# xuhao1/TaichiSLAM

Hardware: AMD Instinct MI355X
Metric: depth-frames/s integrated (640x480->512^3 TSDF) (higher is better)
Workload: dtype f16 storage / f32 + int64 fixed-point arithmetic; 1 GPU; BASELINE configs[1]: single 640x480 u16 depth stream (sphere room r=3 m, 1 deg/frame) -> DenseTSDF 512^3 / 2 cm, recast_step 2, max_ray 5 m; one stream+submap per GPU

## Files before the change

### taichislam_amd/csrc/tsl_integrate.hip

```cpp
#include "tsl_tsdf.hpp"
#include <hip/hip_ext.h>

namespace tsl {

#ifdef TSL_TIMING
#define TSL_T0() const int _wv = (blockIdx.x * (int)blockDim.x + (int)threadIdx.x) >> 6
#define TSL_TICK(F, k) do { long long _n = wall_clock64(); if (lane_id() == 0 && _wv < 16384) (F).dbg[_wv * 16 + (k)] = _n; } while (0)
#else
#define TSL_T0() do {} while (0)
#define TSL_TICK(F, k) do {} while (0)
#endif

#define SCATTER_TILE 4096

struct RayRegs { float pf0, pf1, pf2, d0, d1, d2, P0, P1, P2, w; long long qden; int n; };

__device__ __forceinline__ uint32_t wave_min_u32(uint32_t v)
{
    for (int d = 32; d > 0; d >>= 1) { const uint32_t o = (uint32_t)__shfl_xor((int)v, d); v = o < v ? o : v; }
    return v;
}
__device__ __forceinline__ RayRegs make_ray(const uint4 rec, int n, const FrameParams& P)
{
    RayRegs R;
    R.n = n;
    R.pf0 = h2f((h16)(rec.x & 0xffffu)); R.pf1 = h2f((h16)(rec.x >> 16)); R.pf2 = h2f((h16)(rec.y & 0xffffu));
    R.d0 = h2f((h16)(rec.y >> 16)); R.d1 = h2f((h16)(rec.z & 0xffffu)); R.d2 = h2f((h16)(rec.z >> 16));
    R.w = __uint_as_float(rec.w);
    R.qden = to_fix(R.w);
    R.P0 = R.pf0 + P.T[0]; R.P1 = R.pf1 + P.T[1]; R.P2 = R.pf2 + P.T[2];
    return R;
}
template <bool WITH_N = true>
__device__ __forceinline__ RayRegs load_ray(const FrameDev& F, const FrameParams& P, int r) { return make_ray(F.rayA[r], WITH_N ? F.rayN[r] : 0, P); }
__device__ __forceinline__ void step_voxel(const RayRegs& R, const FrameParams& P, int j, float* x, int* xi)
{
    const float jf = (float)j;
    x[0] = (R.d0 * jf) * P.vs + P.T[0]; x[1] = (R.d1 * jf) * P.vs + P.T[1]; x[2] = (R.d2 * jf) * P.vs + P.T[2];
    xi[0] = rnd_i(div_vs(x[0], P.vs, P.rvs, P.fastdiv)); xi[1] = rnd_i(div_vs(x[1], P.vs, P.rvs, P.fastdiv)); xi[2] = rnd_i(div_vs(x[2], P.vs, P.rvs, P.fastdiv));
}
__device__ __forceinline__ long long step_term(const RayRegs& R, const float* x)
{
    const float v0 = R.P0 - x[0], v1 = R.P1 - x[1], v2 = R.P2 - x[2];
    const float s2 = (v0 * v0 + v1 * v1) + v2 * v2;
    const float dist = s2 >= 1.2621774483536189e-29f ? sqrt_rn_norm(s2) : sqrt_rn(s2);
    const float dot = (v0 * R.pf0 + v1 * R.pf1) + v2 * R.pf2;
    const float sd = dist * (float)sgn_f(dot);
    return to_fix_wave(R.w * sd);
}
template <bool COOP = true>
__device__ __forceinline__ void mark_occupied(const MapDev& M, const FrameParams& P, const RayRegs& R)
{
    const int oi = rnd_i(div_vs(R.P0, P.vs, P.rvs, P.fastdiv)), oj = rnd_i(div_vs(R.P1, P.vs, P.rvs, P.fastdiv)), ok = rnd_i(div_vs(R.P2, P.vs, P.rvs, P.fastdiv));
    if (in_volume(M, oi, oj, ok)) {
        int l; const int b = brick_of(M, oi, oj, ok, &l);
        const int p = pool_claim<COOP>(M, P.slot, b);
        if (p >= 0) M.occ[(size_t)p * TSL_BRK3 + l] = 1;
    }
}
template <bool COOP = true>
__device__ __forceinline__ int frame_slot_slow(const MapDev& M, const FrameDev& F, int s, int b)
{
    const int sl = COOP ? claim_index(F.slot_tab + b, &F.counters[1], F.max_frame_bricks) : claim_index_1(F.slot_tab + b, &F.counters[1], F.max_frame_bricks);
    if (sl >= 0) {
        const int p = pool_claim<COOP>(M, s, b);
        if (p >= 0) { F.touched[sl] = p; F.touched_b[sl] = b; }
        else return -1;
    } else frame_fail(M, F, 2);
// ... 12 lines not shown
    const h16 Tn = f2h((h2f(hmul(T0, W0)) + num) / (h2f(W0) + den));
    float wn = h2f(W0) + den; if (TSL_WMAX < wn) wn = TSL_WMAX;
    return (uint32_t)Tn | ((uint32_t)f2h(wn) << 16);
}
__device__ __forceinline__ uint32_t apply_update_f(uint32_t old, float num, float den)
{
    const h16 T0 = (h16)(old & 0xffffu), W0 = (h16)(old >> 16);
    const h16 Tn = f2h((h2f(hmul(T0, W0)) + num) / (h2f(W0) + den));
    float wn = h2f(W0) + den; if (TSL_WMAX < wn) wn = TSL_WMAX;
    return (uint32_t)Tn | ((uint32_t)f2h(wn) << 16);
}

template <int VARIANT>
__global__ void __launch_bounds__(256) k_integrate(MapDev M, FrameDev F, const FrameParams* __restrict__ Pp)
{
    const FrameParams& P = *Pp;
    const int split = P.split;
    const int gid = blockIdx.x * 256 + threadIdx.x;
    const int r = gid / split, sub = gid - r * split;
    const int nrays = *F.nrays;
    const bool live = r < nrays;
    long long n_ok = 0, n_oob = 0;
    RayRegs R; R.n = 0; R.qden = 0;
    if (live) { R = load_ray(F, P, r); if (sub == 0) mark_occupied(M, P, R); }
    int cur_b = -1; unsigned long long* cur_acc = nullptr;
    int nmax = R.n;
    if (VARIANT == 1) { for (int d = 32; d > 0; d >>= 1) { int o = __shfl_xor(nmax, d); nmax = o > nmax ? o : nmax; } }
    const int iters = (nmax + split - 1) / split;
    for (int it = 0; it < iters; ++it) {
        const int j = 1 + sub + it * split;
        const bool act = live && j <= R.n;
        unsigned long long* dst = nullptr;
        long long qn = 0;
        if (act) {
            float x[3]; int xi[3];
            step_voxel(R, P, j, x, xi);
            if (in_volume(M, xi[0], xi[1], xi[2])) {
                qn = step_term(R, x);
                int l; const int b = brick_of(M, xi[0], xi[1], xi[2], &l);
                if (b != cur_b) { cur_b = b; const int sl = frame_slot(M, F, P.slot, b); cur_acc = sl >= 0 ? F.acc + (size_t)sl * (TSL_BRK3 * 2) : nullptr; }
                if (cur_acc) { dst = cur_acc + (size_t)l * 2; ++n_ok; }
            } else ++n_oob;
        }
        if (VARIANT == 1) {
            const unsigned long long m = __ballot(dst != nullptr);
            if (m) {
                const int leader = (int)__builtin_ctzll(m);
                const unsigned long long lead = __shfl((unsigned long long)dst, leader);
                const bool same = (dst == nullptr) || ((unsigned long long)dst == lead);
                if (__all(same)) {
                    const long long sn = wave_sum_ll(dst ? qn : 0), sdn = wave_sum_ll(dst ? R.qden : 0);
// ... 37 lines not shown
            const int l = q * 256 + threadIdx.x;
            if (a[q].y != 0ull) {
                tw[l] = apply_update(old[q], (long long)a[q].x, (long long)a[q].y);
                obs[l] = 1;
                acc[l] = make_ulonglong2(0ull, 0ull);
                ++uniq;
            }
        }
    }
    for (int sl = blockIdx.x * 256 + threadIdx.x; sl < ntouched; sl += gridDim.x * 256) F.slot_tab[F.touched_b[sl]] = TSL_EMPTY;
    uniq = wave_sum_ll(uniq);
    if (lane_id() == 0 && uniq) atomic_add_i64(&F.stats->unique, uniq);
    if (!list && blockIdx.x == 0 && threadIdx.x == 0) F.stats->bricks = ntouched;
}

__device__ __forceinline__ int axis_coord(float d, float T, const FrameParams& P, int j) { return rnd_i(div_vs((d * (float)j) * P.vs + T, P.vs, P.rvs, P.fastdiv)); }
__device__ __forceinline__ int axis_cell(int c, int h, int N, int nb) { const int u = c + h; return u < 0 ? -1 : (u >= N ? nb : (u >> 4)); }

__device__ __forceinline__ int next_axis_event(float d, float inv_d, float T, const FrameParams& P, float t_over_vs, int j, int jb, int cell, int h, int N, int nb)
{
    if (j >= jb) return jb + 1;
    int bound;
    bool up;
    if (d > 0.0f) { if (cell >= nb) return jb + 1; up = true; bound = (cell < 0 ? 0 : min((cell + 1) * 16, N)) - h; }
    else if (d < 0.0f) { if (cell < 0) return jb + 1; up = false; bound = (cell >= nb ? N - 1 : cell * 16 - 1) - h; }
    else return jb + 1;
    const float est = ((float)bound + (up ? -0.5f : 0.5f) - t_over_vs) * inv_d;
    int e = (int)fminf(fmaxf(ceilf(est), (float)(j + 1)), (float)jb);
    #define TSL_PRED(q) (up ? (axis_coord(d, T, P, (q)) >= bound) : (axis_coord(d, T, P, (q)) <= bound))
    if (TSL_PRED(e)) { while (e - 1 > j && TSL_PRED(e - 1)) --e; }
    else { ++e; while (e <= jb && !TSL_PRED(e)) ++e; }
    #undef TSL_PRED
    return e;
}

#define LH_SIZE 1024
#define LH_EMPTY (-1)
template <int LOG2 = 10>
__device__ __forceinline__ int lh_slot(int* keys, int b)
{
    unsigned h = ((unsigned)b * 2654435761u) >> (32 - LOG2);
    for (int probe = 0; probe < (1 << LOG2); ++probe) {
        const int k = keys[h];
        if (k == b) return (int)h;
        if (k == LH_EMPTY) { const int old = atomicCAS(&keys[h], LH_EMPTY, b); if (old == LH_EMPTY || old == b) return (int)h; }
        h = (h + 1) & ((1u << LOG2) - 1u);
    }
    return -1;
}

#define SEG_RAY_SLOTS 16
#define SEG_LH_LOG2 9
#define SEG_LH (1 << SEG_LH_LOG2)
template <bool FUSED>
__global__ void __launch_bounds__(256) k_segments(MapDev M, BatchDev B)
{
    if ((int)blockIdx.y >= B.n) return;
    const FrameDev& F = B.f[blockIdx.y];
    const FrameParams& P = *B.p[blockIdx.y];
    __shared__ int s_key[SEG_LH];
    __shared__ int s_cnt[SEG_LH];
    TSL_T0();
    TSL_TICK(F, 8);
    for (int i = threadIdx.x; i < SEG_LH; i += 256) { s_key[i] = LH_EMPTY; s_cnt[i] = 0; }
    __syncthreads();
    TSL_TICK(F, 0);

    const int split = P.split;
    const int gid = blockIdx.x * 256 + threadIdx.x;
    const int r = gid / split, sub = gid - r * split;
    const int nrays = FUSED ? F.counters[6] : *F.nrays;
    long long n_ok = 0, n_oob = 0;
    const bool working = __any(r < nrays);
    const int spl = SEG_RAY_SLOTS / split;
    unsigned long long* myseg = F.seg + (size_t)gid * spl;
    int nslot = 0;
    bool ok = r < nrays;
    uint4 rec = make_uint4(0, 0, 0, 0);
    int nsteps = 0;
    if (FUSED) {
        const int lane = threadIdx.x & 63;
        bool big = false;
        int gn = 0, sl = 0;
// ... 11 lines not shown
                uint32_t id[H_INL] = { w0.w, w1.x, w1.y, w1.z, w1.w, w2.x, w2.y, w2.z, w2.w, w3.x, w3.y, w3.z, w3.w };
                uint2 pl[H_INL];
#pragma unroll
                for (int q = 0; q < H_INL; ++q) {
                    if (q >= gn) id[q] = 0xffffffffu;
                    pl[q] = q < gn ? F.pix[id[q]] : make_uint2(0u, 0u);
                }
                PixAcc A = {};
                for (int k = 0; k < gn; ++k) {
                    uint32_t best = 0xffffffffu; uint2 bp = make_uint2(0u, 0u);
#pragma unroll
                    for (int q = 0; q < H_INL; ++q) { const bool t = id[q] < best; best = t ? id[q] : best; bp.x = t ? pl[q].x : bp.x; bp.y = t ? pl[q].y : bp.y; }
#pragma unroll
                    for (int q = 0; q < H_INL; ++q) id[q] = id[q] == best ? 0xffffffffu : id[q];
                    if (k == 0) first = best;
                    if (P.tex) acc_colour(P, F, best, A);
                    acc_payload(bp, A);
                }
                ok = finish_ray(P, F, A, first, &rec, &nsteps);
            }
        }
        for (unsigned long long bm = __ballot(big); bm; bm &= bm - 1ull) {
            const int src = (int)__builtin_ctzll(bm);
            const int n = __shfl(gn, src), sl0 = __shfl(sl, src);
            const unsigned long long vk = ((unsigned long long)(uint32_t)__shfl((int)(vkey >> 32), src) << 32) | (unsigned long long)(uint32_t)__shfl((int)(uint32_t)vkey, src);
            const int nblk = (n + H_INL - 1) / H_INL;
            const uint32_t hmask = (1u << P.hlog2) - 1u;
            auto find_block = [&](int bq) -> int {
                if (bq == 0) return sl0;
                const unsigned long long k2 = h_key(vk, bq);
                uint32_t h = h_hash64(k2, P.hlog2);
                for (uint32_t probe = 0; probe <= hmask; ++probe) {
                    const unsigned long long cur = F.htab[h].key;
                    if (cur == k2) return (int)h;
// ... 11 lines not shown
                uint32_t best = 0xffffffffu;
                for (int bq = lane; bq < nblk; bq += 64) {
                    const int hs = bq == lane ? mine : find_block(bq);
                    if (hs < 0) continue;
                    const int cb = min(H_INL, n - bq * H_INL);
                    const uint32_t* ids = F.htab[hs].pix;
                    for (int q = 0; q < cb; ++q) { const uint32_t v = ids[q]; if ((long long)v > last && v < best) best = v; }
                }
                best = wave_min_u32(best);
                if (best == 0xffffffffu) break;
                if (k == 0) f0 = best;
                acc_pixel(P, F, best, A);
                last = (long long)best;
            }
            uint4 rc; int ns = 0;
            const bool k2 = A.cnt == n && finish_ray(P, F, A, f0, &rc, &ns, lane == src);
            if (lane == src) { rec = rc; nsteps = ns; ok = k2; first = f0; }
        }
        if (r < nrays && sub == 0) {
            F.rayA[r] = rec; F.rayFirst[r] = first;
            if (P.seq) {
                uint32_t u[3];
#pragma unroll
                for (int a = 0; a < 3; ++a) {
                    unsigned long long x = (vkey >> (2 - a)) & 0x1249249249249249ull;
                    x = (x | (x >> 2)) & 0x10c30c30c30c30c3ull; x = (x | (x >> 4)) & 0x100f00f00f00f00full; x = (x | (x >> 8)) & 0x1f0000ff0000ffull;
                    x = (x | (x >> 16)) & 0x1f00000000ffffull; x = (x | (x >> 32)) & 0x1fffffull;
                    u[a] = (uint32_t)x;
                }
                const unsigned long long nblk = (unsigned long long)(P.pcl_ext / P.pcl_blk), blk = (unsigned long long)P.pcl_blk;
                const unsigned long long kb = ((u[0] / P.pcl_blk) * nblk + (u[1] / P.pcl_blk)) * nblk + (u[2] / P.pcl_blk);
                const unsigned long long kl = ((u[0] % P.pcl_blk) * blk + (u[1] % P.pcl_blk)) * blk + (u[2] % P.pcl_blk);
                reinterpret_cast<unsigned long long*>(F.keys)[r] = kb * blk * blk * blk + kl;
                F.rayN[r] = ok ? nsteps : 0;
            }
        }
        block_count_add(&F.stats->v_pcl, r < nrays && sub == 0);
        block_count_add(&F.stats->v_skipped, r < nrays && sub == 0 && !ok);
        if (gid == 0) *F.nrays = nrays;
        const int src = lane - sub;
        rec.x = (uint32_t)__shfl((int)rec.x, src); rec.y = (uint32_t)__shfl((int)rec.y, src); rec.z = (uint32_t)__shfl((int)rec.z, src); rec.w = (uint32_t)__shfl((int)rec.w, src);
        nsteps = __shfl(nsteps, src);
        ok = __shfl((int)ok, src) != 0;
    }
    if (ok) {
        const RayRegs R = FUSED ? make_ray(rec, nsteps, P) : load_ray(F, P, r);
        if (sub == 0) mark_occupied(M, P, R);
        TSL_TICK(F, 1);
        const int len = (R.n + split - 1) / split;
        const int ja = 1 + sub * len, jb = min(R.n, ja + len - 1);
        const float d[3] = { R.d0, R.d1, R.d2 };
        const float id[3] = { __builtin_amdgcn_rcpf(R.d0), __builtin_amdgcn_rcpf(R.d1), __builtin_amdgcn_rcpf(R.d2) };
        const float tv[3] = { P.T[0] / P.vs, P.T[1] / P.vs, P.T[2] / P.vs };
        const int hh[3] = { M.hN, M.hN, M.hNz }, NN[3] = { M.N, M.N, M.Nz }, nb[3] = { M.nbx, M.nbx, M.nbz };
        if (ja <= jb) {
            int cell[3], ev[3];
#pragma unroll
            for (int a = 0; a < 3; ++a) {
                cell[a] = axis_cell(axis_coord(d[a], P.T[a], P, ja), hh[a], NN[a], nb[a]);
                ev[a] = next_axis_event(d[a], id[a], P.T[a], P, tv[a], ja, jb, cell[a], hh[a], NN[a], nb[a]);
            }
            int j = ja;
            while (j <= jb) {
                const int e = min(min(ev[0], ev[1]), ev[2]);
                const bool inside = cell[0] >= 0 && cell[0] < nb[0] && cell[1] >= 0 && cell[1] < nb[1] && cell[2] >= 0 && cell[2] < nb[2];
                if (inside) {
                    const int b = (cell[0] * M.nbx + cell[1]) * M.nbz + cell[2];
                    n_ok += e - j;
                    for (int j0 = j; j0 < e; j0 += SEG_MAX_CNT) {
                        const int cnt = min(e - j0, SEG_MAX_CNT);
                        const unsigned long long en = ((unsigned long long)b << STG_B_SHIFT) | ((unsigned long long)r << (SEG_CNT_BITS + SEG_J_BITS)) |
                                                      ((unsigned long long)j0 << SEG_CNT_BITS) | (unsigned long long)cnt;
                        bool stored = true;
                        if (nslot < spl) myseg[nslot++] = en;
                        else {
// ... 3 lines not shown
                        if (stored) {
                            const int hs = lh_slot<SEG_LH_LOG2>(s_key, b);
                            if (hs >= 0) atomicAdd(&s_cnt[hs], 1);
                            else if (__hip_atomic_fetch_add(&F.bhist[b], 1, __ATOMIC_RELAXED, __HIP_MEMORY_SCOPE_AGENT) == 0) {
                                const int q = __hip_atomic_fetch_add(&F.counters[1], 1, __ATOMIC_RELAXED, __HIP_MEMORY_SCOPE_AGENT);
                                if (q < F.max_frame_bricks) F.act_b[q] = b; else frame_fail(M, F, 2);
                            }
                        }
                    }
                } else n_oob += e - j;
                j = e;
                if (j > jb) break;
#pragma unroll
                for (int a = 0; a < 3; ++a) if (ev[a] == j) {
                    cell[a] += d[a] > 0.0f ? 1 : -1;
                    ev[a] = next_axis_event(d[a], id[a], P.T[a], P, tv[a], j, jb, cell[a], hh[a], NN[a], nb[a]);
                }
            }
        }
    }
    if (r < nrays) for (int q = nslot; q < spl; ++q) myseg[q] = ~0ull;
    TSL_TICK(F, 2);
    __syncthreads();
    TSL_TICK(F, 3);
    TSL_TICK(F, 5);
    for (int i = threadIdx.x; i < SEG_LH; i += 256) {
        const int c = s_cnt[i];
        const int b = c ? s_key[i] : 0;
        const bool first = c && __hip_atomic_fetch_add(&F.bhist[b], c, __ATOMIC_RELAXED, __HIP_MEMORY_SCOPE_AGENT) == 0;
        const int q = wave_reserve(&F.counters[1], first);
        if (first) { if (q < F.max_frame_bricks) F.act_b[q] = b; else frame_fail(M, F, 2); }
// ... 14 lines not shown
        }
        __syncthreads();
        if (threadIdx.x == 0) {
            if (s_steps[0]) atomic_add_i64(&F.stats->steps, s_steps[0]);
            if (s_steps[1]) atomic_add_i64(&F.stats->steps_oob, s_steps[1]);
        }
    }
}

__device__ __forceinline__ int plan_class(int w) { return w >= 2560 ? 0 : (w >= 1280 ? 1 : (w >= 512 ? 2 : 3)); }
__global__ void __launch_bounds__(256) k_plan(MapDev M, BatchDev B, int psegs, int unit_max, int unit_half)
{
    if ((int)blockIdx.y >= B.n) return;
    const int y = blockIdx.y;
    const FrameDev& F = B.f[y];
    const int listed = F.counters[1];
    const int nact = min(listed, F.max_frame_bricks);
    if ((int)blockIdx.x * 256 >= nact && blockIdx.x) return;
    const int i = blockIdx.x * 256 + threadIdx.x;
    int v = 0, b = 0, np = 0, pcls = -1, ucls = -1, tm = 0, wb = 0, tmu = 0, tmp = 0, wu = 0;
    if (i < nact) {
        b = F.act_b[i];
        v = F.bhist[b];
        int vq[TSL_NB];
#pragma unroll
        for (int q = 0; q < TSL_NB; ++q) { vq[q] = q < B.n ? B.f[q].bhist[b] : 0; if (vq[q] > 0) tm |= 1 << q; wb += vq[q]; }
        if (wb > unit_max) { tmp = tm; }
        else if (wb > unit_half) {
            int acc = 0;
#pragma unroll
            for (int q = 0; q < TSL_NB; ++q) if ((tm >> q) & 1) { if (2 * acc < wb) { tmu |= 1 << q; wu += vq[q]; } else tmp |= 1 << q; acc += vq[q]; }
        } else { tmu = tm; wu = wb; }
        if (tmu && (tmu & -tmu) == (1 << y)) ucls = plan_class(wu);
        if (((tmp >> y) & 1) && v > 0) { np = (v + psegs - 1) / psegs; pcls = plan_class((v + np - 1) / np); }
    }
    const int off = block_reserve_n(&F.counters[3], v);
    const int s0 = block_reserve_n(&B.f[0].counters[HDR_SLAB], np);
    int p0 = 0, u0 = 0;
    for (int c = 0; c < PLAN_NCLS; ++c) {
        const int q = block_reserve_n(&F.counters[HDR_PARTS + c], pcls == c ? np : 0); if (pcls == c) p0 = q;
        const int u = block_reserve_n(&B.f[0].counters[HDR_UNITS + c], ucls == c ? 1 : 0); if (ucls == c) u0 = u;
    }
    if (i < nact) {
        F.boffset[b] = off;
        F.bnseg[b] = v;
        const int pool = (np || ucls >= 0) ? pool_claim<false>(M, B.p[y]->slot, b) : -1;
        if (ucls >= 0) {
            if (u0 < B.f[0].unit_cap) B.f[0].unit_tab[(size_t)ucls * B.f[0].unit_cap + u0] = make_int4(b, wu, pool, tmu);
            else for (int q = 0; q < B.n; ++q) if ((tm >> q) & 1) frame_fail(M, B.f[q], 2);
        }
        if (np && pool >= 0) {
            if ((tmp & -tmp) == (1 << y)) {
                const int hi = __hip_atomic_fetch_add(&B.f[0].counters[HDR_HEAVY], 1, __ATOMIC_RELAXED, __HIP_MEMORY_SCOPE_AGENT);
                if (hi < B.f[0].max_frame_bricks) B.f[0].heavy_tab[hi] = make_int4(b, pool, tmp, 0);
                else for (int q = 0; q < B.n; ++q) if ((tm >> q) & 1) frame_fail(M, B.f[q], 2);
            }
            if (s0 + np > F.max_frame_bricks || np >= (1 << PART_NP_BITS) || p0 + np > F.part_cap) frame_fail(M, F, 2);
            else {
                F.bslab[b] = s0 | (np << SLAB_SLOT_BITS);
                const int per = (v + np - 1) / np;
                int4* tab = F.part_tab + (size_t)pcls * F.part_cap;
                for (int k = 0; k < np; ++k) {
                    const int pos = k * per, n = min(v, pos + per) - pos;
                    tab[p0 + k] = make_int4(off + pos, (int)((uint32_t)n | ((uint32_t)np << 16)), pool, s0 + k);
                }
            }
        }
    }
    if (i == 0) { F.stats->bricks = listed; if (listed > F.max_frame_bricks) frame_fail(M, F, 2); }
}

__global__ void __launch_bounds__(256) k_scatter(BatchDev B)
{
    if ((int)blockIdx.y >= B.n) return;
    const FrameDev& F = B.f[blockIdx.y];
    __shared__ int s_key[LH_SIZE];
    __shared__ int s_cnt[LH_SIZE];
    __shared__ int s_base[LH_SIZE];
    if (B.p[blockIdx.y]->group) {
        const int na = F.counters[6], nx = F.counters[7];
        for (int i = blockIdx.x * 256 + threadIdx.x; i < na + nx; i += gridDim.x * 256) {
            HSlot* const hs = F.htab + (i < na ? F.act[i] : F.actx[i - na]);
            hs->key = H_EMPTY; hs->cnt = 0;
        }
    }
    const int total = (int)min((long long)*F.nrays * SEG_RAY_SLOTS + F.counters[2], (long long)F.seg_cap);
    const int ntiles = (total + SCATTER_TILE - 1) / SCATTER_TILE;
    for (int tile = blockIdx.x; tile < ntiles; tile += gridDim.x) {
        for (int i = threadIdx.x; i < LH_SIZE; i += 256) { s_key[i] = LH_EMPTY; s_cnt[i] = 0; }
        __syncthreads();
        const int t0 = tile * SCATTER_TILE;
        unsigned long long key[SCATTER_TILE / 256]; int rank[SCATTER_TILE / 256]; int hs[SCATTER_TILE / 256];
#pragma unroll
        for (int q = 0; q < SCATTER_TILE / 256; ++q) {
            const int i = t0 + q * 256 + threadIdx.x;
            rank[q] = -1; hs[q] = -1;
            if (i < total) {
                key[q] = F.seg[i];
                if (key[q] != ~0ull) {
                    const int b = (int)(key[q] >> STG_B_SHIFT);
                    hs[q] = lh_slot<10>(s_key, b);
                    if (hs[q] >= 0) rank[q] = atomicAdd(&s_cnt[hs[q]], 1);
                    else rank[q] = F.boffset[b] + __hip_atomic_fetch_add(&F.bcursor[b], 1, __ATOMIC_RELAXED, __HIP_MEMORY_SCOPE_AGENT);
                }
            }
        }
        __syncthreads();
        for (int i = threadIdx.x; i < LH_SIZE; i += 256) {
            const int c = s_cnt[i];
            if (c) { const int b = s_key[i]; s_base[i] = F.boffset[b] + __hip_atomic_fetch_add(&F.bcursor[b], c, __ATOMIC_RELAXED, __HIP_MEMORY_SCOPE_AGENT); }
        }
        __syncthreads();
#pragma unroll
        for (int q = 0; q < SCATTER_TILE / 256; ++q)
            if (rank[q] >= 0) F.seg_sorted[(hs[q] >= 0 ? s_base[hs[q]] : 0) + rank[q]] = key[q];
        __syncthreads();
    }
}

#ifdef TSL_NOSWZ
__device__ __forceinline__ int acc_swz5(int l) { return l; }
#else
__device__ __forceinline__ int acc_swz5(int l) { return l ^ (((l >> 8) ^ (l >> 5)) & 31); }
#endif
struct StepK { float vs, rvs, T0, T1, T2; int hN, hNz; };
// ... 188 lines not shown
        if (threadIdx.x < 64) s_bin[threadIdx.x] = 0;
        __syncthreads();
        TSL_PRIME(0, f)
    }
    uint32_t old[VPT];
    uint32_t vmask = 0u;
    bool have_old = false;
    for (;;) {
        const int* const it = s_it[slot];
        const int slot1 = slot == 2 ? 0 : slot + 1, slot2 = slot == 0 ? 2 : slot - 1;
        const bool unit = uni(it[IT_UNIT]) != 0;
        const int p = uni(it[IT_POOL]), rk = uni(it[IT_SLAB]);
        const uint32_t fmask = (uint32_t)uni(it[IT_FMASK]);
        const int n_f = uni(it[IT_N + f]);
        const FrameDev& F = B.f[f];
        const FrameParams& P = *B.p[f];
        const StepK K = { P.vs, P.rvs, P.T[0], P.T[1], P.T[2], M.hN, M.hNz };
        const uint32_t later = fmask >> (f + 1);
        const bool first_frame = (fmask & ((1u << f) - 1u)) == 0u, last_frame = later == 0u;
        const bool first_step = first_frame && c == 0;
        const int nseg = min(CSEGS, n_f - c * CSEGS);
        const bool last_chunk = (c + 1) * CSEGS >= n_f;
        const bool last_step = last_chunk && last_frame;
        int known = max(1, (n_f + CSEGS - 1) / CSEGS) - 1 - c + steps_of(slot, later << (f + 1));
        if (n_known >= 1) known += steps_of(slot1, (uint32_t)uni(s_it[slot1][IT_FMASK]));
        const bool do_claim = !exhausted && n_known < 2 && known <= 1;
        if (do_claim && threadIdx.x == 0) s_claim[0] = __hip_atomic_fetch_add(claim, 1, __ATOMIC_RELAXED, __HIP_MEMORY_SCOPE_AGENT);
#ifdef TSL_TIMING
        long long* const _rec = F.dbg + 131072 + (size_t)blockIdx.x * 128 + (size_t)(t < 16 ? t : 15) * 8;
        if (threadIdx.x == 0 && first_step) { _rec[0] = wall_clock64(); _rec[1] = (unit ? 1 : 0) | (uni(it[IT_NP]) << 8) | ((long long)fmask << 32); _rec[2] = 0; _rec[5] = 0; }
        if (threadIdx.x == 0 && c == 0) _rec[2] += n_f;
// ... 15 lines not shown
#pragma unroll
        for (int q = 0; q < SPT; ++q) { const int i = q * NT + threadIdx.x; kn[q] = i < nsegn ? Fx.seg_sorted[offx + i] : 0ull; }
        const uint32_t* const twr = M.tw + (size_t)(p >= 0 ? p : 0) * TSL_BRK3;
        if (first_step) { have_old = false; vmask = 0u; }
        if (!TEX && unit && p >= 0 && first_step) {
#pragma unroll
            for (int q = 0; q < VPT; ++q) old[q] = twr[q * NT + threadIdx.x];
            have_old = true;
        }
#pragma unroll
        for (int q = 0; q < SPT; ++q) {
            const int i = q * NT + ((q & 1) ? NT - 1 - (int)threadIdx.x : (int)threadIdx.x);
            if (i >= nseg) continue;
            const unsigned long long key = kk[q];
            const int cnt = (int)(key & ((1u << SEG_CNT_BITS) - 1)), j0 = (int)((key >> SEG_CNT_BITS) & ((1u << SEG_J_BITS) - 1));
            const RayRegs R = make_ray(recs[q], 0, P);
            const uint32_t wid = wids[q];
#ifndef TSL_EXP_STAGGER
#define TSL_EXP_STAGGER 27
#endif
            int off = ((int)((threadIdx.x * (unsigned)TSL_EXP_STAGGER) & 63u) * cnt) >> 6;
            for (int s = 0; s < cnt; s += 2) {
                const int ja = j0 + off; off = (off + 1 == cnt) ? 0 : off + 1;
                const int jb = j0 + off; off = (off + 1 == cnt) ? 0 : off + 1;
                int la, lb; float qa, qb;
                step_eval<FASTDIV>(R, K, ja, &la, &qa);
                step_eval<FASTDIV>(R, K, jb, &lb, &qb);
                long long na = (long long)(int)qa, nb = (long long)(int)qb;
                if (__builtin_expect(__any(!(fabsf(qa) < 2147483648.0f) || !(fabsf(qb) < 2147483648.0f)), 0)) { na = __float2ll_rn(qa); nb = __float2ll_rn(qb); }
                atomicAdd(&S_NUM(la), (unsigned long long)na);
                atomicAdd(&S_DEN(la), (unsigned long long)R.qden);
// ... 218 lines not shown
}

int check_variant2(tsl_tsdf* m)
{
    TSL_REQUIRE(m->F.max_frame_bricks <= 4096 && m->P.max_steps_f < (float)(1 << SEG_J_BITS) && m->F.max_points < (1 << STG_RAY_BITS) && m->nb3 < (1 << 24) && 3 * m->pcl_bits <= H_BLOCK_SHIFT,
                "variant 2: ray too long / too many points / too many bricks for the segment key (use variant 1)");
    return TSL_OK;
}

int launch_segments(tsl_tsdf* m, const BatchDev& B, const FrameParams* hp, int total, hipStream_t st)
{
    const FrameParams& P = hp[0];
    if (P.variant != 2) return TSL_OK;
    const int iblocks = (int)(((int64_t)total * P.split + 255) / 256);
    prof_begin(m, TSL_K_SEGMENTS, st);
    if (P.group) hipLaunchKernelGGL(k_segments<true>, dim3(iblocks, B.n), dim3(256), 0, st, m->M, B);
    else hipLaunchKernelGGL(k_segments<false>, dim3(iblocks, B.n), dim3(256), 0, st, m->M, B);
    prof_end(m, st);
    int unit_max = m->unit_max <= m->unit_floor ? m->unit_max : std::max(m->unit_floor, (int)((long long)m->unit_max * B.n / TSL_NB));
    int unit_half = std::min(unit_max, m->unit_half <= 2048 ? m->unit_half : std::max(2048, (int)((long long)m->unit_half * B.n / TSL_NB)));
    if (P.seq && m->seq_impl) unit_max = unit_half = 1 << 30;
    prof_begin(m, TSL_K_BIN, st);
    hipLaunchKernelGGL(k_plan, dim3((B.f[0].max_frame_bricks + 255) / 256, B.n), dim3(256), 0, st, m->M, B, m->chunks * m->wg * m->spt, unit_max, unit_half);
    hipLaunchKernelGGL(k_scatter, dim3(256, B.n), dim3(256), 0, st, B);
    prof_end(m, st);
    return TSL_OK;
}

int launch_brick(tsl_tsdf* m, const BatchDev& B, const FrameParams& P, int kind, hipStream_t st, hipEvent_t start, hipEvent_t stop)
{
    const int bg = kind == 2 ? m->pgrid : (B.n <= 2 ? (m->bgrid + 1) / 2 : (kind == 1 ? m->ugrid : m->bgrid));
#define TSL_LAUNCH_IB(TEXV, FD) do { \
        if (m->wg == 512 && m->spt == 2 && !TEXV) hipExtLaunchKernelGGL((k_integrate_batch<false, FD, 512, 2, 4>), dim3((2 * m->ncu * bg + 99) / 100), dim3(512), 0, st, start, stop, 0, m->M, B, kind); \
        else if (m->wg == 512) hipExtLaunchKernelGGL((k_integrate_batch<TEXV, FD, 512, 4, 2>), dim3((m->ncu * bg + 99) / 100), dim3(512), 0, st, start, stop, 0, m->M, B, kind); \
        else hipExtLaunchKernelGGL((k_integrate_batch<TEXV, FD, 256, 4, (TEXV ? 1 : 2)>), dim3(((TEXV ? 1 : 2) * m->ncu * bg + 99) / 100), dim3(256), 0, st, start, stop, 0, m->M, B, kind); } while (0)
    if (P.tex) { if (P.fastdiv) TSL_LAUNCH_IB(true, true); else TSL_LAUNCH_IB(true, false); }
    else { if (P.fastdiv) TSL_LAUNCH_IB(false, true); else TSL_LAUNCH_IB(false, false); }
#undef TSL_LAUNCH_IB
    TSL_HIP(hipGetLastError());
// ... 35 lines not shown
```

### taichislam_amd/csrc/tsl_tsdf.hip

```cpp
#include "tsl_tsdf.hpp"
#include <rocprim/rocprim.hpp>
#include <algorithm>
#include <cmath>
#include <cstdio>
#include <cstdlib>
#include <cstring>
#include <mutex>

namespace tsl {

static thread_local std::string g_err;
void set_error(const std::string& s) { g_err = s; }

__device__ __forceinline__ uint32_t part1by2_32(uint32_t x)
{
    x &= 0x3ffu;
    x = (x ^ (x << 16)) & 0xff0000ffu;
    x = (x ^ (x << 8)) & 0x0300f00fu;
    x = (x ^ (x << 4)) & 0x030c30c3u;
    x = (x ^ (x << 2)) & 0x09249249u;
    return x;
}
__device__ __forceinline__ uint64_t part1by2_64(uint64_t x)
{
// ... 123 lines not shown
    const FrameParams& P = *Pp;
    const int total = P.total;
    const int i = blockIdx.x * 256 + threadIdx.x;
    const K bad = KeyOps<K>::invalid(P.pcl_bits);
    bool head = false, ok = false;
    uint4 rec = make_uint4(0, 0, 0, 0);
    int nsteps = 0;
    uint32_t first = 0;
    if (i < total) {
        const K k = keys_s[i];
        head = (k != bad) && (i == 0 || keys_s[i - 1] != k);
        if (head) {
            PixAcc A = {};
            first = F.vals_s[i];
            for (int q = i; q < total && keys_s[q] == k; ++q) acc_pixel(P, F, F.vals_s[q], A);
            ok = finish_ray(P, F, A, first, &rec, &nsteps);
        }
    }
    const int r = block_reserve(F.nrays, ok);
    if (ok) { F.rayA[r] = rec; F.rayN[r] = nsteps; F.rayFirst[r] = first; }
    block_count_add(&F.stats->v_pcl, head);
    block_count_add(&F.stats->v_skipped, head && !ok);
}

__device__ __forceinline__ int group_insert(const FrameDev& F, unsigned long long vkey, bool inside, uint32_t pid, int log2n, bool* opened, int* xslot)
{
    HSlot* const tab = F.htab;
    const uint32_t mask = (1u << log2n) - 1u;
    const int lane = lane_id();
    const uint32_t klo = (uint32_t)vkey, khi = (uint32_t)(vkey >> 32);
    int leader = lane, grank = 0, gsize = 1;
// ... 355 lines not shown
    if (!serial && m->esdf_gate_set) {
        TSL_HIP(hipStreamWaitEvent(sa, m->esdf_gate_ev, 0));
        m->esdf_gate_mask |= 1u << (bi % TSL_NSTREAMS);
        if (m->esdf_gate_mask == (1u << TSL_NSTREAMS) - 1u) m->esdf_gate_set = false;
    }
    for (int k = 0; k < m->nproducers; ++k) {
        if (m->producers[k] == sa) continue;
        if (hipStreamQuery(m->producers[k]) == hipSuccess) continue;
        if (!m->in_ev[0]) for (auto& e : m->in_ev) TSL_HIP(hipEventCreateWithFlags(&e, hipEventDisableTiming));
        hipEvent_t e = m->in_ev[m->in_ev_next]; m->in_ev_next = (m->in_ev_next + 1) % 8;
        TSL_HIP(hipEventRecord(e, m->producers[k]));
        TSL_HIP(hipStreamWaitEvent(sa, e, 0));
    }
    m->nproducers = 0;
    BatchDev B; ParamPack PP;
    for (int q = 0; q < n; ++q) { FSet& S = m->fset[bi * TSL_NB + q]; B.f[q] = S.F; B.p[q] = S.Pd; PP.p[q] = m->pend[q]; }
    for (int q = n; q < TSL_NB; ++q) { B.f[q] = B.f[0]; B.p[q] = B.p[0]; PP.p[q] = PP.p[0]; }
    B.n = n;
    SetPtrs SP;
    for (int q = 0; q < TSL_NB; ++q) { SP.p[q] = const_cast<FrameParams*>(B.p[q]); SP.header[q] = reinterpret_cast<int*>(B.f[q].stats); }
    hipLaunchKernelGGL(k_set_params, dim3(n), dim3(64), 0, sa, PP, SP);
    {
        StageCopy C; int most = 0; bool any_host = false;
        for (int q = 0; q < TSL_NB; ++q) {
            FSet& S = m->fset[bi * TSL_NB + q];
            const bool on = q < n;
            C.src[2 * q] = static_cast<const uint4*>(S.pin_dev); C.dst[2 * q] = static_cast<uint4*>(S.stage_in); C.n16[2 * q] = on ? (int)((S.copy_in + 15) / 16) : 0;
            C.src[2 * q + 1] = reinterpret_cast<const uint4*>(static_cast<const char*>(S.pin_dev) + S.copy_tex_off); C.dst[2 * q + 1] = static_cast<uint4*>(S.stage_tex); C.n16[2 * q + 1] = on ? (int)((S.copy_tex + 15) / 16) : 0;
            most = std::max(most, std::max(C.n16[2 * q], C.n16[2 * q + 1]));
            any_host = any_host || C.n16[2 * q] || C.n16[2 * q + 1];
            if (on) { S.copy_in = 0; S.copy_tex = 0; }
        }
// ... 977 lines not shown
```

### taichislam_amd/csrc/tsl_tsdf.hpp

```cpp
#pragma once
#include "tsl_common.hpp"

namespace tsl {

struct FrameParams {
    float R[9], T[3];
    float fx, fy, cx, cy;
    float fxc, fyc, cxc, cyc;
    float vs;
    float rvs; int fastdiv;
    float thr_max, thr_min;
    float max_ray_f;
    float max_steps_f;
    float internal_f;
    int   pcl_lo, pcl_ext, pcl_bits;
    int   step, hh, ww, H, W;
    int   rstride;
    int   cstride;
    int   th, tw, tex, same_proj;
    int   slot;
    int   variant, split;
    int   group;
    int   seq, pcl_blk;
    int   hlog2;
    const void* input; int total;
    const uint8_t* tex_input; int points;
};

struct FrameDev {
    uint32_t *keys, *keys_s, *vals, *vals_s;
    uint2* pix;
    uint4* rayA;
    int*   rayN;
    uint32_t* rayFirst;
    struct HSlot* htab; int hlog2;
    int*   act;
    int*   actx;
    uint2* colpix;
    tsl_frame_stats* stats;
    int*   nrays;
    int*   counters;
    unsigned long long *seg, *seg_sorted;
// ... 69 lines not shown
    }
    A.cr = hadd(A.cr, f2h((float)rgb[0])); A.cg = hadd(A.cg, f2h((float)rgb[1])); A.cb = hadd(A.cb, f2h((float)rgb[2]));
}
__device__ __forceinline__ void acc_payload(const uint2 pl, PixAcc& A)
{
    A.sx = hadd(A.sx, (h16)(pl.x & 0xffffu)); A.sy = hadd(A.sy, (h16)(pl.x >> 16));
    A.sz = hadd(A.sz, (h16)(pl.y & 0xffffu)); A.zs = hadd(A.zs, (h16)(pl.y >> 16));
    ++A.cnt;
}
__device__ __forceinline__ void acc_pixel(const FrameParams& P, const FrameDev& F, uint32_t pid, PixAcc& A)
{
    if (P.tex) acc_colour(P, F, pid, A);
    acc_payload(F.pix[pid], A);
}

__device__ __forceinline__ bool finish_ray(const FrameParams& P, const FrameDev& F, const PixAcc& A, uint32_t first, uint4* rec, int* nsteps, bool write_colour = true)
{
    const h16 c = f2h((float)A.cnt);
    const h16 px = hdiv(A.sx, c), py = hdiv(A.sy, c), pz = hdiv(A.sz, c);
    const h16 len = hsqrt(hadd(hadd(hmul(px, px), hmul(py, py)), hmul(pz, pz)));
    const h16 zbar = hdiv(A.zs, c);
    const float lenf = h2f(len), zzf = h2f(hmul(zbar, zbar));
    if (!((lenf > 0.0f) && isfinite(lenf) && (zzf > 0.0f) && isfinite(zzf))) return false;
    const h16 dx = hdiv(px, len), dy = hdiv(py, len), dz = hdiv(pz, len);
    float nf = lenf / P.vs + P.internal_f;
    if (P.max_steps_f < nf) nf = P.max_steps_f;
    *nsteps = (int)nf;
    float w = 1.0f / zzf;
    if (w > TSL_W_CLAMP) w = TSL_W_CLAMP;
    rec->x = (uint32_t)px | ((uint32_t)py << 16);
    rec->y = (uint32_t)pz | ((uint32_t)dx << 16);
// ... 22 lines not shown

struct ProfSlot { hipEvent_t a, b; int kid; int count; };

#define TSL_NB 8
#define TSL_NBATCH 3
#define TSL_NSTREAMS 3
#define TSL_NSETS (TSL_NB * TSL_NBATCH)
struct FSet {
    FrameDev F; void* sort_temp; void* header; size_t header_bytes;
    void* stage_in; size_t stage_in_bytes; void* stage_tex; size_t stage_tex_bytes;
    void* pin; size_t pin_bytes; void* pin_dev;
    size_t copy_in, copy_tex, copy_tex_off;
    FrameParams* Pd;
    std::vector<void*> owned;
};
struct BatchDev { FrameDev f[TSL_NB]; const FrameParams* p[TSL_NB]; int n; };
struct ParamPack { FrameParams p[TSL_NB]; };
struct SetPtrs { FrameParams* p[TSL_NB]; int* header[TSL_NB]; };
struct BatchHost { hipStream_t st; hipEvent_t a_done, b_done, p_done, c_done; bool b_pending, a_recorded, c_recorded; };
struct StageCopy { const uint4* src[2 * TSL_NB]; uint4* dst[2 * TSL_NB]; int n16[2 * TSL_NB]; };
#define TSL_INFLIGHT 8

int fuse_submaps_sequential(tsl_tsdf* g, tsl_tsdf* sub, const float* pose_dev, int nsrc);
int esdf_finish(tsl_tsdf* m);
void esdf_release(tsl_tsdf* m);
struct FrontierState;
void frontier_release(tsl_tsdf* m);
}

#define TSL_ESDF_SLOTS 4
struct EsdfSlot { hipEvent_t ev; int* host; int rounds; tsl_esdf_stats st; };
// ... 86 lines not shown
```

Baseline: 34480 frames/s.

## Cache frame params in registers/kernel args, batch plan reservations, template fastdiv

Copies the per-frame parameters used in hot loops into a compact register struct (RayK) and passes pose/voxel size through kernel arguments (FrameK), so inner loops no longer reload them through a global pointer. The segments kernel is specialised on fastdiv at compile time. k_plan replaces its many per-counter block reservations with a single multi-counter wave scan followed by one atomic per counter. k_scatter batches its cursor atomics and takes the group flag as a kernel argument. The cost is more template instantiations and larger kernel arguments, checked by a static_assert.

```diff
diff --git a/taichislam_amd/csrc/tsl_integrate.hip b/taichislam_amd/csrc/tsl_integrate.hip
--- a/taichislam_amd/csrc/tsl_integrate.hip
+++ b/taichislam_amd/csrc/tsl_integrate.hip
@@ -20,7 +20,7 @@
     for (int d = 32; d > 0; d >>= 1) { const uint32_t o = (uint32_t)__shfl_xor((int)v, d); v = o < v ? o : v; }
     return v;
 }
-__device__ __forceinline__ RayRegs make_ray(const uint4 rec, int n, const FrameParams& P)
+__device__ __forceinline__ RayRegs make_ray(const uint4 rec, int n, float T0, float T1, float T2)
 {
     RayRegs R;
     R.n = n;
@@ -28,16 +28,16 @@
     R.d0 = h2f((h16)(rec.y >> 16)); R.d1 = h2f((h16)(rec.z & 0xffffu)); R.d2 = h2f((h16)(rec.z >> 16));
     R.w = __uint_as_float(rec.w);
     R.qden = to_fix(R.w);
-    R.P0 = R.pf0 + P.T[0]; R.P1 = R.pf1 + P.T[1]; R.P2 = R.pf2 + P.T[2];
+    R.P0 = R.pf0 + T0; R.P1 = R.pf1 + T1; R.P2 = R.pf2 + T2;
     return R;
 }
 template <bool WITH_N = true>
-__device__ __forceinline__ RayRegs load_ray(const FrameDev& F, const FrameParams& P, int r) { return make_ray(F.rayA[r], WITH_N ? F.rayN[r] : 0, P); }
-__device__ __forceinline__ void step_voxel(const RayRegs& R, const FrameParams& P, int j, float* x, int* xi)
+__device__ __forceinline__ RayRegs load_ray(const FrameDev& F, const RayK& K, int r) { return make_ray(F.rayA[r], WITH_N ? F.rayN[r] : 0, K.T[0], K.T[1], K.T[2]); }
+__device__ __forceinline__ void step_voxel(const RayRegs& R, const RayK& K, int fast, int j, float* x, int* xi)
 {
     const float jf = (float)j;
-    x[0] = (R.d0 * jf) * P.vs + P.T[0]; x[1] = (R.d1 * jf) * P.vs + P.T[1]; x[2] = (R.d2 * jf) * P.vs + P.T[2];
-    xi[0] = rnd_i(div_vs(x[0], P.vs, P.rvs, P.fastdiv)); xi[1] = rnd_i(div_vs(x[1], P.vs, P.rvs, P.fastdiv)); xi[2] = rnd_i(div_vs(x[2], P.vs, P.rvs, P.fastdiv));
+    x[0] = (R.d0 * jf) * K.vs + K.T[0]; x[1] = (R.d1 * jf) * K.vs + K.T[1]; x[2] = (R.d2 * jf) * K.vs + K.T[2];
+    xi[0] = rnd_i(div_vs(x[0], K.vs, K.rvs, fast)); xi[1] = rnd_i(div_vs(x[1], K.vs, K.rvs, fast)); xi[2] = rnd_i(div_vs(x[2], K.vs, K.rvs, fast));
 }
 __device__ __forceinline__ long long step_term(const RayRegs& R, const float* x)
 {
@@ -49,9 +49,9 @@
     return to_fix_wave(R.w * sd);
 }
 template <bool COOP = true>
-__device__ __forceinline__ void mark_occupied(const MapDev& M, const FrameParams& P, const RayRegs& R)
-{
-    const int oi = rnd_i(div_vs(R.P0, P.vs, P.rvs, P.fastdiv)), oj = rnd_i(div_vs(R.P1, P.vs, P.rvs, P.fastdiv)), ok = rnd_i(div_vs(R.P2, P.vs, P.rvs, P.fastdiv));
+__device__ __forceinline__ void mark_occupied(const MapDev& M, const RayK& P, int fast, const RayRegs& R)
+{
+    const int oi = rnd_i(div_vs(R.P0, P.vs, P.rvs, fast)), oj = rnd_i(div_vs(R.P1, P.vs, P.rvs, fast)), ok = rnd_i(div_vs(R.P2, P.vs, P.rvs, fast));
     if (in_volume(M, oi, oj, ok)) {
         int l; const int b = brick_of(M, oi, oj, ok, &l);
         const int p = pool_claim<COOP>(M, P.slot, b);
@@ -94,7 +94,8 @@
 template <int VARIANT>
 __global__ void __launch_bounds__(256) k_integrate(MapDev M, FrameDev F, const FrameParams* __restrict__ Pp)
 {
-    const FrameParams& P = *Pp;
+    const RayK P = ray_k(*Pp);
+    const int fast = Pp->fastdiv;
     const int split = P.split;
     const int gid = blockIdx.x * 256 + threadIdx.x;
     const int r = gid / split, sub = gid - r * split;
@@ -102,7 +103,7 @@
     const bool live = r < nrays;
     long long n_ok = 0, n_oob = 0;
     RayRegs R; R.n = 0; R.qden = 0;
-    if (live) { R = load_ray(F, P, r); if (sub == 0) mark_occupied(M, P, R); }
+    if (live) { R = load_ray(F, P, r); if (sub == 0) mark_occupied(M, P, fast, R); }
     int cur_b = -1; unsigned long long* cur_acc = nullptr;
     int nmax = R.n;
     if (VARIANT == 1) { for (int d = 32; d > 0; d >>= 1) { int o = __shfl_xor(nmax, d); nmax = o > nmax ? o : nmax; } }
@@ -114,7 +115,7 @@
         long long qn = 0;
         if (act) {
             float x[3]; int xi[3];
-            step_voxel(R, P, j, x, xi);
+            step_voxel(R, P, fast, j, x, xi);
             if (in_volume(M, xi[0], xi[1], xi[2])) {
                 qn = step_term(R, x);
                 int l; const int b = brick_of(M, xi[0], xi[1], xi[2], &l);
@@ -182,10 +183,12 @@
     if (!list && blockIdx.x == 0 && threadIdx.x == 0) F.stats->bricks = ntouched;
 }
 
-__device__ __forceinline__ int axis_coord(float d, float T, const FrameParams& P, int j) { return rnd_i(div_vs((d * (float)j) * P.vs + T, P.vs, P.rvs, P.fastdiv)); }
+template <bool FASTDIV>
+__device__ __forceinline__ int axis_coord(float d, float T, float vs, float rvs, int j) { return rnd_i(div_vs((d * (float)j) * vs + T, vs, rvs, FASTDIV ? 1 : 0)); }
 __device__ __forceinline__ int axis_cell(int c, int h, int N, int nb) { const int u = c + h; return u < 0 ? -1 : (u >= N ? nb : (u >> 4)); }
 
-__device__ __forceinline__ int next_axis_event(float d, float inv_d, float T, const FrameParams& P, float t_over_vs, int j, int jb, int cell, int h, int N, int nb)
+template <bool FASTDIV>
+__device__ __forceinline__ int next_axis_event(float d, float inv_d, float T, float vs, float rvs, float t_over_vs, int j, int jb, int cell, int h, int N, int nb)
 {
     if (j >= jb) return jb + 1;
     int bound;
@@ -195,7 +198,7 @@
     else return jb + 1;
     const float est = ((float)bound + (up ? -0.5f : 0.5f) - t_over_vs) * inv_d;
     int e = (int)fminf(fmaxf(ceilf(est), (float)(j + 1)), (float)jb);
-    #define TSL_PRED(q) (up ? (axis_coord(d, T, P, (q)) >= bound) : (axis_coord(d, T, P, (q)) <= bound))
+    #define TSL_PRED(q) (up ? (axis_coord<FASTDIV>(d, T, vs, rvs, (q)) >= bound) : (axis_coord<FASTDIV>(d, T, vs, rvs, (q)) <= bound))
     if (TSL_PRED(e)) { while (e - 1 > j && TSL_PRED(e - 1)) --e; }
     else { ++e; while (e <= jb && !TSL_PRED(e)) ++e; }
     #undef TSL_PRED
@@ -220,12 +223,14 @@
 #define SEG_RAY_SLOTS 16
 #define SEG_LH_LOG2 9
 #define SEG_LH (1 << SEG_LH_LOG2)
-template <bool FUSED>
+template <bool FUSED, bool FASTDIV>
 __global__ void __launch_bounds__(256) k_segments(MapDev M, BatchDev B)
 {
     if ((int)blockIdx.y >= B.n) return;
     const FrameDev& F = B.f[blockIdx.y];
-    const FrameParams& P = *B.p[blockIdx.y];
+    const FrameParams P = *B.p[blockIdx.y];
+    const RayK K = ray_k(P);
+    constexpr int fast = FASTDIV ? 1 : 0;
     __shared__ int s_key[SEG_LH];
     __shared__ int s_cnt[SEG_LH];
     TSL_T0();
@@ -234,7 +239,7 @@
     __syncthreads();
     TSL_TICK(F, 0);
 
-    const int split = P.split;
+    const int split = K.split;
     const int gid = blockIdx.x * 256 + threadIdx.x;
     const int r = gid / split, sub = gid - r * split;
     const int nrays = FUSED ? F.counters[6] : *F.nrays;
@@ -276,10 +281,10 @@
 #pragma unroll
                     for (int q = 0; q < H_INL; ++q) id[q] = id[q] == best ? 0xffffffffu : id[q];
                     if (k == 0) first = best;
-                    if (P.tex) acc_colour(P, F, best, A);
+                    if (K.tex) acc_colour(P, F, best, A);
                     acc_payload(bp, A);
                 }
-                ok = finish_ray(P, F, A, first, &rec, &nsteps);
+                ok = finish_ray(K, F, A, first, &rec, &nsteps);
             }
         }
         for (unsigned long long bm = __ballot(big); bm; bm &= bm - 1ull) {
@@ -321,12 +326,12 @@
                 last = (long long)best;
             }
             uint4 rc; int ns = 0;
-            const bool k2 = A.cnt == n && finish_ray(P, F, A, f0, &rc, &ns, lane == src);
+            const bool k2 = A.cnt == n && finish_ray(K, F, A, f0, &rc, &ns, lane == src);
             if (lane == src) { rec = rc; nsteps = ns; ok = k2; first = f0; }
         }
         if (r < nrays && sub == 0) {
             F.rayA[r] = rec; F.rayFirst[r] = first;
-            if (P.seq) {
+            if (K.seq) {
                 uint32_t u[3];
 #pragma unroll
                 for (int a = 0; a < 3; ++a) {
@@ -351,21 +356,21 @@
         ok = __shfl((int)ok, src) != 0;
     }
     if (ok) {
-        const RayRegs R = FUSED ? make_ray(rec, nsteps, P) : load_ray(F, P, r);
-        if (sub == 0) mark_occupied(M, P, R);
+        const RayRegs R = FUSED ? make_ray(rec, nsteps, K.T[0], K.T[1], K.T[2]) : load_ray(F, K, r);
+        if (sub == 0) mark_occupied(M, K, fast, R);
         TSL_TICK(F, 1);
         const int len = (R.n + split - 1) / split;
         const int ja = 1 + sub * len, jb = min(R.n, ja + len - 1);
         const float d[3] = { R.d0, R.d1, R.d2 };
         const float id[3] = { __builtin_amdgcn_rcpf(R.d0), __builtin_amdgcn_rcpf(R.d1), __builtin_amdgcn_rcpf(R.d2) };
-        const float tv[3] = { P.T[0] / P.vs, P.T[1] / P.vs, P.T[2] / P.vs };
+        const float tv[3] = { K.T[0] / K.vs, K.T[1] / K.vs, K.T[2] / K.vs };
         const int hh[3] = { M.hN, M.hN, M.hNz }, NN[3] = { M.N, M.N, M.Nz }, nb[3] = { M.nbx, M.nbx, M.nbz };
         if (ja <= jb) {
             int cell[3], ev[3];
 #pragma unroll
             for (int a = 0; a < 3; ++a) {
-                cell[a] = axis_cell(axis_coord(d[a], P.T[a], P, ja), hh[a], NN[a], nb[a]);
-                ev[a] = next_axis_event(d[a], id[a], P.T[a], P, tv[a], ja, jb, cell[a], hh[a], NN[a], nb[a]);
+                cell[a] = axis_cell(axis_coord<FASTDIV>(d[a], K.T[a], K.vs, K.rvs, ja), hh[a], NN[a], nb[a]);
+                ev[a] = next_axis_event<FASTDIV>(d[a], id[a], K.T[a], K.vs, K.rvs, tv[a], ja, jb, cell[a], hh[a], NN[a], nb[a]);
             }
             int j = ja;
             while (j <= jb) {
@@ -399,7 +404,7 @@
 #pragma unroll
                 for (int a = 0; a < 3; ++a) if (ev[a] == j) {
                     cell[a] += d[a] > 0.0f ? 1 : -1;
-                    ev[a] = next_axis_event(d[a], id[a], P.T[a], P, tv[a], j, jb, cell[a], hh[a], NN[a], nb[a]);
+                    ev[a] = next_axis_event<FASTDIV>(d[a], id[a], K.T[a], K.vs, K.rvs, tv[a], j, jb, cell[a], hh[a], NN[a], nb[a]);
                 }
             }
         }
@@ -444,6 +449,7 @@
     if ((int)blockIdx.y >= B.n) return;
     const int y = blockIdx.y;
     const FrameDev& F = B.f[y];
+    const int slot = B.p[y]->slot;
     const int listed = F.counters[1];
     const int nact = min(listed, F.max_frame_bricks);
     if ((int)blockIdx.x * 256 >= nact && blockIdx.x) return;
@@ -464,17 +470,39 @@
         if (tmu && (tmu & -tmu) == (1 << y)) ucls = plan_class(wu);
         if (((tmp >> y) & 1) && v > 0) { np = (v + psegs - 1) / psegs; pcls = plan_class((v + np - 1) / np); }
     }
-    const int off = block_reserve_n(&F.counters[3], v);
-    const int s0 = block_reserve_n(&B.f[0].counters[HDR_SLAB], np);
+    constexpr int NCTR = 2 + 2 * PLAN_NCLS;
+    __shared__ int s_w[NCTR][4];
+    __shared__ int s_b[NCTR];
+    const int lane = lane_id(), wid = threadIdx.x >> 6;
+    int cnt[NCTR], inc[NCTR];
+    cnt[0] = v; cnt[1] = np;
+#pragma unroll
+    for (int c = 0; c < PLAN_NCLS; ++c) { cnt[2 + c] = pcls == c ? np : 0; cnt[2 + PLAN_NCLS + c] = ucls == c ? 1 : 0; }
+#pragma unroll
+    for (int k = 0; k < NCTR; ++k) {
+        inc[k] = cnt[k];
+        for (int d = 1; d < 64; d <<= 1) { const int o = __shfl_up(inc[k], d); if (lane >= d) inc[k] += o; }
+        if (lane == 63) s_w[k][wid] = inc[k];
+    }
+    __syncthreads();
+    if (threadIdx.x < NCTR) {
+        const int k = threadIdx.x;
+        const int tot = s_w[k][0] + s_w[k][1] + s_w[k][2] + s_w[k][3];
+        int* const ctr = k == 0 ? &F.counters[3] : (k == 1 ? &B.f[0].counters[HDR_SLAB] : (k < 2 + PLAN_NCLS ? &F.counters[HDR_PARTS + k - 2] : &B.f[0].counters[HDR_UNITS + k - 2 - PLAN_NCLS]));
+        s_b[k] = tot ? __hip_atomic_fetch_add(ctr, tot, __ATOMIC_RELAXED, __HIP_MEMORY_SCOPE_AGENT) : 0;
+    }
+    __syncthreads();
+    int first[NCTR];
+#pragma unroll
+    for (int k = 0; k < NCTR; ++k) { first[k] = s_b[k] + inc[k] - cnt[k]; for (int w = 0; w < wid; ++w) first[k] += s_w[k][w]; }
+    const int off = first[0], s0 = first[1];
     int p0 = 0, u0 = 0;
-    for (int c = 0; c < PLAN_NCLS; ++c) {
-        const int q = block_reserve_n(&F.counters[HDR_PARTS + c], pcls == c ? np : 0); if (pcls == c) p0 = q;
-        const int u = block_reserve_n(&B.f[0].counters[HDR_UNITS + c], ucls == c ? 1 : 0); if (ucls == c) u0 = u;
-    }
+#pragma unroll
+    for (int c = 0; c < PLAN_NCLS; ++c) { if (pcls == c) p0 = first[2 + c]; if (ucls == c) u0 = first[2 + PLAN_NCLS + c]; }
     if (i < nact) {
         F.boffset[b] = off;
         F.bnseg[b] = v;
-        const int pool = (np || ucls >= 0) ? pool_claim<false>(M, B.p[y]->slot, b) : -1;
+        const int pool = (np || ucls >= 0) ? pool_claim<false>(M, slot, b) : -1;
         if (ucls >= 0) {
             if (u0 < B.f[0].unit_cap) B.f[0].unit_tab[(size_t)ucls * B.f[0].unit_cap + u0] = make_int4(b, wu, pool, tmu);
             else for (int q = 0; q < B.n; ++q) if ((tm >> q) & 1) frame_fail(M, B.f[q], 2);
@@ -500,14 +528,14 @@
     if (i == 0) { F.stats->bricks = listed; if (listed > F.max_frame_bricks) frame_fail(M, F, 2); }
 }
 
-__global__ void __launch_bounds__(256) k_scatter(BatchDev B)
+__global__ void __launch_bounds__(256) k_scatter(BatchDev B, int group)
 {
     if ((int)blockIdx.y >= B.n) return;
     const FrameDev& F = B.f[blockIdx.y];
     __shared__ int s_key[LH_SIZE];
     __shared__ int s_cnt[LH_SIZE];
     __shared__ int s_base[LH_SIZE];
-    if (B.p[blockIdx.y]->group) {
+    if (group) {
         const int na = F.counters[6], nx = F.counters[7];
         for (int i = blockIdx.x * 256 + threadIdx.x; i < na + nx; i += gridDim.x * 256) {
             HSlot* const hs = F.htab + (i < na ? F.act[i] : F.actx[i - na]);
@@ -536,9 +564,17 @@
             }
         }
         __syncthreads();
-        for (int i = threadIdx.x; i < LH_SIZE; i += 256) {
-            const int c = s_cnt[i];
-            if (c) { const int b = s_key[i]; s_base[i] = F.boffset[b] + __hip_atomic_fetch_add(&F.bcursor[b], c, __ATOMIC_RELAXED, __HIP_MEMORY_SCOPE_AGENT); }
+        {
+            constexpr int NE = LH_SIZE / 256;
+            int c[NE], b[NE], bo[NE], at[NE];
+#pragma unroll
+            for (int q = 0; q < NE; ++q) { const int i = q * 256 + threadIdx.x; c[q] = s_cnt[i]; b[q] = c[q] ? s_key[i] : 0; }
+#pragma unroll
+            for (int q = 0; q < NE; ++q) bo[q] = c[q] ? F.boffset[b[q]] : 0;
+#pragma unroll
+            for (int q = 0; q < NE; ++q) at[q] = c[q] ? __hip_atomic_fetch_add(&F.bcursor[b[q]], c[q], __ATOMIC_RELAXED, __HIP_MEMORY_SCOPE_AGENT) : 0;
+#pragma unroll
+            for (int q = 0; q < NE; ++q) if (c[q]) s_base[q * 256 + threadIdx.x] = bo[q] + at[q];
         }
         __syncthreads();
 #pragma unroll
@@ -757,7 +793,7 @@
         const uint32_t fmask = (uint32_t)uni(it[IT_FMASK]);
         const int n_f = uni(it[IT_N + f]);
         const FrameDev& F = B.f[f];
-        const FrameParams& P = *B.p[f];
+        const FrameK& P = B.k[f];
         const StepK K = { P.vs, P.rvs, P.T[0], P.T[1], P.T[2], M.hN, M.hNz };
         const uint32_t later = fmask >> (f + 1);
         const bool first_frame = (fmask & ((1u << f) - 1u)) == 0u, last_frame = later == 0u;
@@ -803,7 +839,7 @@
             if (i >= nseg) continue;
             const unsigned long long key = kk[q];
             const int cnt = (int)(key & ((1u << SEG_CNT_BITS) - 1)), j0 = (int)((key >> SEG_CNT_BITS) & ((1u << SEG_J_BITS) - 1));
-            const RayRegs R = make_ray(recs[q], 0, P);
+            const RayRegs R = make_ray(recs[q], 0, K.T0, K.T1, K.T2);
             const uint32_t wid = wids[q];
 #ifndef TSL_EXP_STAGGER
 #define TSL_EXP_STAGGER 27
@@ -1052,15 +1088,17 @@
     if (P.variant != 2) return TSL_OK;
     const int iblocks = (int)(((int64_t)total * P.split + 255) / 256);
     prof_begin(m, TSL_K_SEGMENTS, st);
-    if (P.group) hipLaunchKernelGGL(k_segments<true>, dim3(iblocks, B.n), dim3(256), 0, st, m->M, B);
-    else hipLaunchKernelGGL(k_segments<false>, dim3(iblocks, B.n), dim3(256), 0, st, m->M, B);
+#define TSL_LAUNCH_SEG(G, FD) hipLaunchKernelGGL((k_segments<G, FD>), dim3(iblocks, B.n), dim3(256), 0, st, m->M, B)
+    if (P.group) { if (P.fastdiv) TSL_LAUNCH_SEG(true, true); else TSL_LAUNCH_SEG(true, false); }
+    else { if (P.fastdiv) TSL_LAUNCH_SEG(false, true); else TSL_LAUNCH_SEG(false, false); }
+#undef TSL_LAUNCH_SEG
     prof_end(m, st);
     int unit_max = m->unit_max <= m->unit_floor ? m->unit_max : std::max(m->unit_floor, (int)((long long)m->unit_max * B.n / TSL_NB));
     int unit_half = std::min(unit_max, m->unit_half <= 2048 ? m->unit_half : std::max(2048, (int)((long long)m->unit_half * B.n / TSL_NB)));
     if (P.seq && m->seq_impl) unit_max = unit_half = 1 << 30;
     prof_begin(m, TSL_K_BIN, st);
     hipLaunchKernelGGL(k_plan, dim3((B.f[0].max_frame_bricks + 255) / 256, B.n), dim3(256), 0, st, m->M, B, m->chunks * m->wg * m->spt, unit_max, unit_half);
-    hipLaunchKernelGGL(k_scatter, dim3(256, B.n), dim3(256), 0, st, B);
+    hipLaunchKernelGGL(k_scatter, dim3(256, B.n), dim3(256), 0, st, B, P.group);
     prof_end(m, st);
     return TSL_OK;
 }
diff --git a/taichislam_amd/csrc/tsl_tsdf.hip b/taichislam_amd/csrc/tsl_tsdf.hip
--- a/taichislam_amd/csrc/tsl_tsdf.hip
+++ b/taichislam_amd/csrc/tsl_tsdf.hip
@@ -161,7 +161,7 @@
             PixAcc A = {};
             first = F.vals_s[i];
             for (int q = i; q < total && keys_s[q] == k; ++q) acc_pixel(P, F, F.vals_s[q], A);
-            ok = finish_ray(P, F, A, first, &rec, &nsteps);
+            ok = finish_ray(ray_k(P), F, A, first, &rec, &nsteps);
         }
     }
     const int r = block_reserve(F.nrays, ok);
@@ -547,8 +547,12 @@
     }
     m->nproducers = 0;
     BatchDev B; ParamPack PP;
-    for (int q = 0; q < n; ++q) { FSet& S = m->fset[bi * TSL_NB + q]; B.f[q] = S.F; B.p[q] = S.Pd; PP.p[q] = m->pend[q]; }
-    for (int q = n; q < TSL_NB; ++q) { B.f[q] = B.f[0]; B.p[q] = B.p[0]; PP.p[q] = PP.p[0]; }
+    for (int q = 0; q < n; ++q) {
+        FSet& S = m->fset[bi * TSL_NB + q]; B.f[q] = S.F; B.p[q] = S.Pd; PP.p[q] = m->pend[q];
+        const FrameParams& Pq = m->pend[q];
+        B.k[q] = FrameK{ { Pq.T[0], Pq.T[1], Pq.T[2] }, Pq.vs, Pq.rvs };
+    }
+    for (int q = n; q < TSL_NB; ++q) { B.f[q] = B.f[0]; B.p[q] = B.p[0]; B.k[q] = B.k[0]; PP.p[q] = PP.p[0]; }
     B.n = n;
     SetPtrs SP;
     for (int q = 0; q < TSL_NB; ++q) { SP.p[q] = const_cast<FrameParams*>(B.p[q]); SP.header[q] = reinterpret_cast<int*>(B.f[q].stats); }
diff --git a/taichislam_amd/csrc/tsl_tsdf.hpp b/taichislam_amd/csrc/tsl_tsdf.hpp
--- a/taichislam_amd/csrc/tsl_tsdf.hpp
+++ b/taichislam_amd/csrc/tsl_tsdf.hpp
@@ -26,6 +26,16 @@
     const void* input; int total;
     const uint8_t* tex_input; int points;
 };
+
+struct RayK { float T[3], vs, rvs, internal_f, max_steps_f; int split, seq, tex, slot; };
+__device__ __forceinline__ RayK ray_k(const FrameParams& P)
+{
+    RayK K;
+    K.T[0] = P.T[0]; K.T[1] = P.T[1]; K.T[2] = P.T[2]; K.vs = P.vs; K.rvs = P.rvs; K.internal_f = P.internal_f; K.max_steps_f = P.max_steps_f;
+    K.split = P.split; K.seq = P.seq; K.tex = P.tex; K.slot = P.slot;
+    return K;
+}
+struct FrameK { float T[3], vs, rvs; };
 
 struct FrameDev {
     uint32_t *keys, *keys_s, *vals, *vals_s;
@@ -125,7 +135,7 @@
     acc_payload(F.pix[pid], A);
 }
 
-__device__ __forceinline__ bool finish_ray(const FrameParams& P, const FrameDev& F, const PixAcc& A, uint32_t first, uint4* rec, int* nsteps, bool write_colour = true)
+__device__ __forceinline__ bool finish_ray(const RayK& P, const FrameDev& F, const PixAcc& A, uint32_t first, uint4* rec, int* nsteps, bool write_colour = true)
 {
     const h16 c = f2h((float)A.cnt);
     const h16 px = hdiv(A.sx, c), py = hdiv(A.sy, c), pz = hdiv(A.sz, c);
@@ -178,7 +188,8 @@
     FrameParams* Pd;
     std::vector<void*> owned;
 };
-struct BatchDev { FrameDev f[TSL_NB]; const FrameParams* p[TSL_NB]; int n; };
+struct BatchDev { FrameDev f[TSL_NB]; const FrameParams* p[TSL_NB]; FrameK k[TSL_NB]; int n; };
+static_assert(sizeof(MapDev) + sizeof(BatchDev) + 64 <= 4096, "the batch kernels' arguments must fit 4 KiB");
 struct ParamPack { FrameParams p[TSL_NB]; };
 struct SetPtrs { FrameParams* p[TSL_NB]; int* header[TSL_NB]; };
 struct BatchHost { hipStream_t st; hipEvent_t a_done, b_done, p_done, c_done; bool b_pending, a_recorded, c_recorded; };
```

Result: slower. 33660 frames/s (-2.4%).
